# KyleVanMeter/MVOLPS

Hardware: AMD Instinct MI355X
Metric: simplex_pivots_per_s (higher is better)
Workload: dtype f64

## Files before the change

### include/mvx.h

```cpp
#ifndef MVX_H
#define MVX_H

#ifdef __cplusplus
extern "C" {
#endif

#define MVX_MIN 1
#define MVX_MAX 2
#define MVX_CV 1
#define MVX_IV 2
#define MVX_BV 3
#define MVX_FR 1
#define MVX_LO 2
#define MVX_UP 3
#define MVX_DB 4
#define MVX_FX 5
#define MVX_BS 1
#define MVX_NL 2
#define MVX_NU 3
#define MVX_NF 4
#define MVX_NS 5
#define MVX_UNDEF 1
#define MVX_FEAS 2
#define MVX_INFEAS 3
// ... 100 lines not shown
int mvx_price_cols(const mvx_prob *P, int k, const double *cols, const double *obj, double *dj, double *img);
int mvx_price_cols_tile(void);
void mvx_set_mat_col(mvx_prob *P, int j, int len, const int *ind, const double *val);
int mvx_get_mat_col(const mvx_prob *P, int j, int *ind, double *val);
int mvx_del_cols(mvx_prob *P, int ncs, const int *num);
int mvx_del_cols_span(void);
int mvx_conflict_graph(const mvx_prob *model, unsigned long long *adj, long long *edges);
int mvx_polish_many(const mvx_prob *root, int count, double *x, int max_moves, double *obj, int *moves, int *ok);

int mvx_get_tableau_ld(const mvx_prob *P);
int mvx_get_tableau(const mvx_prob *P, double *out);
int mvx_get_basis(const mvx_prob *P, int *head, int *nb, int *flag);

int mvx_device_count(void);
int mvx_set_device(int dev);
void mvx_profile_enable(int on);
void mvx_profile_reset(void);
double mvx_profile_update_ms(void);
long long mvx_profile_update_launches(void);
double mvx_last_solve_ms(const mvx_prob *P);
long long mvx_pack_size(const mvx_prob *P);
int mvx_pack(const mvx_prob *P, void *dev_buf);
long long mvx_pack_size_from(const mvx_prob *P, const mvx_prob *base);
int mvx_pack_from(const mvx_prob *P, const mvx_prob *base, void *dev_buf);
int mvx_unpack(mvx_prob *dst, const mvx_prob *base, const void *dev_buf);
void mvx_set_tuning(int tr, int hot, int nt);
void mvx_set_refresh(int check_every, double tol);
int mvx_get_refresh_cnt(const mvx_prob *P);
double mvx_row_residual(const mvx_prob *P);
void mvx_set_persist(int mode);
void mvx_set_chain(int len);
void mvx_set_cluster(int on);
void mvx_cluster_stats(long long *launches, long long *aborts);
void mvx_set_dual_chain(int len);
void mvx_persist_stats(long long *launches, long long *aborts);
void mvx_persist_cycles(unsigned long long *out5);
void mvx_set_batch_slots(int slots);
void mvx_sync(void);
int mvx_last_error(void);
int mvx_bind_thread(void);

#ifdef __cplusplus
}
#endif
#endif
```

### mvolps_amd/__init__.py

```python
import ctypes as C
import os

from . import capi

_HERE = os.path.dirname(os.path.abspath(__file__))
LIB_PATH = os.path.join(_HERE, "lib", "libmvolps_amd.so")

_EXTRA = {
    "del_rows": (C.c_int, [C.c_void_p, C.c_int, C.POINTER(C.c_int)]),
    "del_rows_many": (C.c_int, [C.c_void_p, C.c_int, C.POINTER(C.c_int), C.POINTER(C.c_int)]),
    "add_cut_rows_many": (C.c_int, [C.c_void_p, C.c_int, C.POINTER(C.c_int), C.POINTER(C.c_double), C.POINTER(C.c_double)]),
    "ranges": (C.c_int, [C.c_void_p, C.POINTER(C.c_double), C.POINTER(C.c_int)]),
    "ranges_chunk": (C.c_int, []),
    "add_dense_cols": (C.c_int, [C.c_void_p, C.c_int, C.POINTER(C.c_double), C.POINTER(C.c_double), C.POINTER(C.c_int),
                                 C.POINTER(C.c_double), C.POINTER(C.c_double), C.POINTER(C.c_int)]),
    "price_cols": (C.c_int, [C.c_void_p, C.c_int, C.POINTER(C.c_double), C.POINTER(C.c_double), C.POINTER(C.c_double),
                             C.POINTER(C.c_double)]),
    "price_cols_tile": (C.c_int, []),
    "del_cols": (C.c_int, [C.c_void_p, C.c_int, C.POINTER(C.c_int)]),
    "del_cols_span": (C.c_int, []),
    "set_mat_col": (None, [C.c_void_p, C.c_int, C.c_int, C.POINTER(C.c_int), C.POINTER(C.c_double)]),
    "get_mat_col": (C.c_int, [C.c_void_p, C.c_int, C.POINTER(C.c_int), C.POINTER(C.c_double)]),
    "device_count": (C.c_int, []),
    "set_device": (C.c_int, [C.c_int]),
    "profile_enable": (None, [C.c_int]),
    "profile_reset": (None, []),
    "profile_update_ms": (C.c_double, []),
    "profile_update_launches": (C.c_longlong, []),
    "last_solve_ms": (C.c_double, [C.c_void_p]),
    "sync": (None, []),
    "set_tuning": (None, [C.c_int, C.c_int, C.c_int]),
    "set_batch_slots": (None, [C.c_int]),
    "set_persist": (None, [C.c_int]),
    "set_chain": (None, [C.c_int]),
    "set_cluster": (None, [C.c_int]),
    "cluster_stats": (None, [C.POINTER(C.c_longlong), C.POINTER(C.c_longlong)]),
    "set_dual_chain": (None, [C.c_int]),
    "set_refresh": (None, [C.c_int, C.c_double]),
    "get_refresh_cnt": (C.c_int, [C.c_void_p]),
    "row_residual": (C.c_double, [C.c_void_p]),
    "persist_stats": (None, [C.POINTER(C.c_longlong), C.POINTER(C.c_longlong)]),
    "last_error": (C.c_int, []),
    "bind_thread": (C.c_int, []),
    "persist_cycles": (None, [C.POINTER(C.c_ulonglong)]),
    "simplex_batch": (C.c_int, [C.POINTER(C.c_void_p), C.c_int, C.c_void_p, C.POINTER(C.c_int)]),
    "pack_size": (C.c_longlong, [C.c_void_p]),
    "pack": (C.c_int, [C.c_void_p, C.c_void_p]),
    "pack_size_from": (C.c_longlong, [C.c_void_p, C.c_void_p]),
    "pack_from": (C.c_int, [C.c_void_p, C.c_void_p, C.c_void_p]),
    "unpack": (C.c_int, [C.c_void_p, C.c_void_p, C.c_void_p]),
}

_api = None


def load_library():
    if os.environ.get("MVX_NO_TORCH") != "1":
        try:
            import torch
        except Exception:
            pass
    if not os.path.exists(LIB_PATH):
        raise RuntimeError(
            "libmvolps_amd.so is missing (%s): build it with `python -m mvolps_amd.build`; "
            "there is no fallback path" % LIB_PATH
        )
    return C.CDLL(LIB_PATH)


# ... 19 lines not shown
```

### mvolps_amd/csrc/capi.cpp

```cpp
#include <algorithm>
#include <cfloat>
#include <cmath>
#include <cstdio>
#include <cstdlib>
#include <chrono>
#include <cstring>

#include "engine.hpp"
#include "../../include/mvx_dist.h"

using mvx::RowPtr;

static const double INF = HUGE_VAL;
static int g_term_out = 1;

static void fault(const char *msg) {
  std::fprintf(stderr, "mvx: %s\n", msg);
  std::abort();
}

static void norm_bounds(int type, double lb, double ub, double *olb, double *oub) {
  switch (type) {
    case MVX_FR: *olb = -INF; *oub = INF; break;
    case MVX_LO: *olb = lb; *oub = INF; break;
// ... 722 lines not shown
int mvx_conflict_graph(const mvx_prob *model, unsigned long long *adj, long long *edges) {
  return mvx::engine_conflict_graph(model, adj, edges);
}
int mvx_polish_many(const mvx_prob *root, int count, double *x, int max_moves, double *obj, int *moves, int *ok) {
  return mvx::engine_polish_many(root, count, x, max_moves, obj, moves, ok);
}

int mvx_device_count(void) { return mvx::device_count(); }
int mvx_set_device(int dev) { return mvx::set_device(dev); }
long long mvx_pack_size(const mvx_prob *P) { return mvx::engine_pack_size(P, P->m); }
int mvx_pack(const mvx_prob *P, void *dev_buf) { return mvx::engine_pack(P, P->m, dev_buf); }
long long mvx_pack_size_from(const mvx_prob *P, const mvx_prob *base) { return mvx::engine_pack_size(P, base ? base->m : P->m); }
int mvx_pack_from(const mvx_prob *P, const mvx_prob *base, void *dev_buf) { return mvx::engine_pack(P, base ? base->m : P->m, dev_buf); }
int mvx_unpack(mvx_prob *dst, const mvx_prob *base, const void *dev_buf) {
  if (dst == base) return -1;
  mvx::release_device(dst);
  dst->m = base->m; dst->n = base->n; dst->dir = base->dir;
  dst->A = base->A; dst->c = base->c; dst->kind = base->kind; dst->cname = base->cname;
  dst->rtype = base->rtype; dst->rlb = base->rlb; dst->rub = base->rub;
  dst->ctype = base->ctype; dst->clb = base->clb; dst->cub = base->cub;
  dst->valid = false; dst->sol_fresh = false; dst->fresh_rows = -1;
  return mvx::engine_unpack(dst, dev_buf);
}
void mvx_set_tuning(int tr, int hot, int nt) { mvx::tuning(tr, hot, nt); }
void mvx_set_stall_limit(int limit) { mvx::set_stall_limit(limit); }
int mvx_fcs_debug_stamps(unsigned long long *out) { return mvx::fcs_debug_stamps(out); }
void mvx_set_refresh(int check_every, double tol) { mvx::set_refresh(check_every, tol); }
int mvx_get_refresh_cnt(const mvx_prob *P) { return P->refresh_cnt; }
double mvx_row_residual(const mvx_prob *P) { return mvx::row_residual(P); }
void mvx_set_persist(int mode) { mvx::set_persist(mode); }
void mvx_set_chain(int len) { mvx::set_chain(len); }
void mvx_set_cluster(int on) { mvx::set_cluster(on); }
void mvx_cluster_stats(long long *launches, long long *aborts) { mvx::cluster_stats(launches, aborts); }
void mvx_set_dual_chain(int len) { mvx::set_dual_chain(len); }
void mvx_persist_stats(long long *launches, long long *aborts) { mvx::persist_stats(launches, aborts); }
void mvx_persist_cycles(unsigned long long *out5) { mvx::persist_cycles(out5); }
void mvx_set_batch_slots(int slots) { mvx::set_batch_slots(slots); }
void mvx_profile_enable(int on) { mvx::profile_enable(on); }
void mvx_profile_reset(void) { mvx::profile_reset(); }
double mvx_profile_update_ms(void) { return mvx::profile_update_ms(); }
long long mvx_profile_update_launches(void) { return mvx::profile_update_launches(); }
double mvx_last_solve_ms(const mvx_prob *P) { return P->last_ms; }
void mvx_sync(void) { mvx::sync_stream(); }
int mvx_last_error(void) { return mvx::take_last_error(); }
int mvx_bind_thread(void) { return mvx::bind_thread(); }

void *mvx_image_alloc(size_t bytes) { return mvx::engine_image_alloc(bytes); }
void mvx_image_free(void *buf) { mvx::engine_image_free(buf); }
static long long img_pack_size(const void *P, const void *base) { return mvx_pack_size_from((const mvx_prob *)P, (const mvx_prob *)base); }
static int img_pack(const void *P, const void *base, void *buf) { return mvx_pack_from((const mvx_prob *)P, (const mvx_prob *)base, buf); }
static int img_unpack(void *dst, const void *base, const void *buf) { return mvx_unpack((mvx_prob *)dst, (const mvx_prob *)base, buf); }
const mvx_image_api *mvx_hip_image_api(void) {
  static const mvx_image_api t = {img_pack_size, img_pack, img_unpack, mvx_image_alloc, mvx_image_free};
  return &t;
}

}
```

### mvolps_amd/csrc/engine.cpp

```cpp
#include <hip/hip_runtime.h>

#include <algorithm>
#include <cmath>
#include <cstdio>
#include <cstdlib>
#include <cstring>
#include <atomic>
#include <functional>
#include <limits>
#include <map>
#include <mutex>
#include <tuple>
#include <unordered_map>
#include <unordered_set>
#include <vector>

#include "engine.hpp"

struct DevMatrix {
  int m0 = 0, n = 0, lda = 0;
  double *plain = nullptr, *packed = nullptr;
  int *len = nullptr;
  std::vector<const void *> rows;
  ~DevMatrix() {
// ... 637 lines not shown
    *ub = P->rub[k];
  } else {
    *lb = P->clb[k - P->m];
    *ub = P->cub[k - P->m];
  }
}

static std::atomic<int> g_cluster{-1};
static std::atomic<bool> g_cluster_broken{false};
static std::atomic<long long> g_cluster_launches{0}, g_cluster_aborts{0};
static bool cluster_wanted() {
  int v = g_cluster.load();
  if (v < 0) {
    const char *e = std::getenv("MVX_CLUSTER");
    v = e ? (std::atoi(e) != 0) : 1;
    g_cluster.store(v);
  }
  return v != 0 && !g_cluster_broken.load();
}

static int g_chain = -1;
static int chain_length(const mvx_prob *P) {
  if (g_chain < 0) {
    const char *e = std::getenv("MVX_CHAIN");
    g_chain = e ? std::max(1, std::min(KCH, std::atoi(e))) : 0;
  }
  if (g_chain > 0) return g_chain;
  const size_t bytes = (size_t)(P->m + 1) * (size_t)P->ld * 8;
  if (cluster_wanted() && chain_cluster_kmax(P->m, P->n) > 0) return bytes < ((size_t)24 << 20) ? 16 : 32;
  if (bytes < ((size_t)24 << 20)) return 8;
  return 16;
}

static int g_dchain = -1;
static int dual_chain_length(bool wide, bool on_chip = false) {
  if (g_dchain < 0) {
    const char *e = std::getenv("MVX_DCHAIN");
    g_dchain = e ? std::max(1, std::min(DCH_MAX, std::atoi(e))) : 0;
  }
  if (g_dchain > 0) return g_dchain;
  if (on_chip) return 8;
  return wide ? 8 : 4;
}

static int pivot_budget(const mvx_prob *P, const mvx_smcp &parm) {
  return parm.it_lim >= 0 ? parm.it_lim : 200 * (P->m + P->n) + 100000;
}

static void ctl_for_handle(Ctl *h, const mvx_prob *P, double tol_bnd, double tol_dj, double tol_piv, int budget) {
  std::memset(h, 0, sizeof(Ctl));
  h->T = P->d_T;
  h->bvar = P->d_bvar; h->blb = P->d_blb; h->bub = P->d_bub;
  h->nvar = P->d_nvar; h->nflag = P->d_nflag; h->nlb = P->d_nlb; h->nub = P->d_nub;
  h->m = P->m; h->n = P->n; h->ld = P->ld; h->m_cap = P->m_cap;
  h->sgn = (P->dir == MVX_MAX) ? 1.0 : -1.0;
  h->tol_bnd = tol_bnd; h->tol_dj = tol_dj; h->tol_piv = tol_piv;
  h->phase = PH_START; h->done = D_RUN; h->budget = budget;
  h->stall = 0; h->stall_limit = g_stall_limit > 0 ? g_stall_limit : 64 + (P->m + P->n) / 8;
  h->fstate = F_OFF;
  h->nch = 1;
}

static void fill_ctl(SolveCtx &sc, mvx_prob *P, Ctl *h, const mvx_smcp *parm = nullptr) {
  if (parm) ctl_for_handle(h, P, parm->tol_bnd, parm->tol_dj, parm->tol_piv, pivot_budget(P, *parm));
  else ctl_for_handle(h, P, 1e-9, 1e-9, 1e-9, -1);
  h->colq = sc.d_colq; h->srow = sc.d_srow; h->cost1 = sc.d_cost1; h->wts = sc.d_wts;
// ... 132 lines not shown
        double acc = 0.0;
        if (any_x)
          for (int j = 1; j <= n; j++)
            if (xn[j] != 0.0) acc = std::fma(a[j], xn[j], acc);
        row[0] = acc;
      }
    }
    HIPCHECK(hipMemcpyAsync(P->d_T + r0 * ld, bounce, (r1 - r0) * ld * 8, hipMemcpyHostToDevice, sc.stream));
    HIPCHECK(hipStreamSynchronize(sc.stream));
  }
  HIPCHECK(hipHostFree(bounce));
  HIPCHECK(hipMemcpyAsync(P->d_bvar, P->bvar.data(), (size_t)(m + 1) * 4, hipMemcpyHostToDevice, sc.stream));
  HIPCHECK(hipMemcpyAsync(P->d_blb, blb.data(), (size_t)(m + 1) * 8, hipMemcpyHostToDevice, sc.stream));
  HIPCHECK(hipMemcpyAsync(P->d_bub, bub.data(), (size_t)(m + 1) * 8, hipMemcpyHostToDevice, sc.stream));
  std::vector<int> nv((size_t)ld, 0), nf((size_t)ld, MVX_NS);
  for (int j = 1; j <= n; j++) {
    nv[j] = P->nvar[j];
    nf[j] = P->nflag[j];
  }
  HIPCHECK(hipMemcpyAsync(P->d_nvar, nv.data(), (size_t)ld * 4, hipMemcpyHostToDevice, sc.stream));
  HIPCHECK(hipMemcpyAsync(P->d_nflag, nf.data(), (size_t)ld * 4, hipMemcpyHostToDevice, sc.stream));
  HIPCHECK(hipMemcpyAsync(P->d_nlb, nlb.data(), (size_t)ld * 8, hipMemcpyHostToDevice, sc.stream));
  HIPCHECK(hipMemcpyAsync(P->d_nub, nub.data(), (size_t)ld * 8, hipMemcpyHostToDevice, sc.stream));
  HIPCHECK(hipStreamSynchronize(sc.stream));
  rebuild_pos(P);
  P->pending.clear();
  P->valid = true;
  P->sol_fresh = false;
  P->fresh_rows = -1;
  P->status = MVX_UNDEF;
  return true;
}

static void flush_update_events(Context &c, size_t used) {
  for (size_t k = 0; k + 1 < used; k += 2) {
    float ms = 0.f;
    HIPCHECK(hipEventElapsedTime(&ms, c.ev_pool[k], c.ev_pool[k + 1]));
    c.prof_update_ms += ms;
    c.prof_update_n++;
  }
}

constexpr int PERSIST_HEAD_STRIDE_MAX = 4;
static std::atomic<int> g_persist_mode{-1};
static std::atomic<bool> g_persist_broken{false};
static std::atomic<long long> g_persist_launches{0}, g_persist_aborts{0};
struct PersistPlan {
  int cpw = 0, nw = 0;
  size_t lds = 0;
};
static bool persist_plan(Context &c, const mvx_prob *P, PersistPlan *pl) {
  if (g_persist_broken) return false;
  if (g_persist_mode < 0) {
    const char *e = std::getenv("MVX_PERSIST");
    g_persist_mode = (e && e[0] == '0') ? 0 : ((e && e[0] == '2') ? 2 : 1);
  }
  if (!g_persist_mode) return false;
  static int cus = 0;
  if (!cus) {
    hipDeviceProp_t prop;
    if (hipGetDeviceProperties(&prop, c.dev) != hipSuccess) return false;
    cus = prop.multiProcessorCount;
  }
  const int m = P->m, n = P->n;
  if ((long)(m + 1) * (n + 1) < 32768) return false;
  if (g_persist_mode < 2 && (long)(m + 1) * (n + 1) > 700000) return false;
  const int cpw = (n + cus - 1) / cus;
  if (cpw > persist_max_cpw()) return false;
// ... 14 lines not shown
    HIPCHECK(hipMalloc((void **)&sc.d_pcand, (size_t)2 * 256 * PERSIST_HEAD_STRIDE_MAX * 8));
    HIPCHECK(hipMalloc((void **)&sc.d_pctl, sizeof(Ctl)));
  }
  if (words > sc.p_msg_words) {
    HIPCHECK(hipStreamSynchronize(sc.stream));
    if (sc.d_pmsg) HIPCHECK(hipFree(sc.d_pmsg));
    HIPCHECK(hipMalloc((void **)&sc.d_pmsg, (size_t)2 * 256 * words * 8));
    sc.p_msg_words = words;
  }
  if (P->ld > sc.p_pw_ld) {
    HIPCHECK(hipStreamSynchronize(sc.stream));
    if (sc.d_ppw) HIPCHECK(hipFree(sc.d_ppw));
    HIPCHECK(hipMalloc((void **)&sc.d_ppw, (size_t)2 * P->ld * 8));
    sc.p_pw_ld = P->ld;
  }
  if (sc.p_backup_bytes != P->slab_bytes) {
    if (sc.p_backup) slab_recycle(c, sc.p_backup, sc.p_backup_bytes);
    sc.p_backup = slab_alloc(c, P->slab_bytes);
    sc.p_backup_bytes = sc.p_backup ? P->slab_bytes : 0;
    if (!sc.p_backup) {
      (void)g_last_error.exchange(0);
      return false;
    }
  }
  return true;
}

struct SolveJob {
  mvx_prob *P = nullptr;
  SolveCtx *sc = nullptr;
  mvx_smcp parm;
  enum { MAIN, PHASE1, FINAL } mode = MAIN;
  int batch = 8, pb = 4;
  int done = D_RUN;
  bool try_fused = false;
  bool try_dfused = false;
  bool persist_queued = false;
  int seen_steps = 0, seen_pivots = 0, seen_bulk = 0;
  int chain = 1, chain0 = 1;
  bool resident = false;
  bool cluster = false;
  ChainArgs cargs{};
  size_t ev_used = 0;
  bool profiled = false;
  int rc = 0;
  Ctl snap;
};

static void stage_copy_async(SolveCtx &sc, const mvx_prob *P) {
  HIPCHECK(hipEventRecord(sc.ev_b, sc.stream));
  if (!sc.stage_zc) HIPCHECK(hipMemcpyAsync(sc.h_stage, sc.d_stage, StageView::bytes(P->m_cap, P->ld), hipMemcpyDeviceToHost, sc.stream));
  if (sc.d_pabort) HIPCHECK(hipMemcpyAsync(sc.h_pabort, sc.d_pabort, 512, hipMemcpyDeviceToHost, sc.stream));
}

static bool dual_fused_worth_it(const mvx_prob *P) {
  static int mode = -1;
  if (mode < 0) {
    const char *e = std::getenv("MVX_DUAL_FUSED");
    mode = e ? std::atoi(e) : 1;
  }
  if (mode == 0) return false;
  if (mode >= 2) return true;
  const long entries = (long)(P->m + 1) * (P->n + 1);
  return entries >= 2000000 && entries < 12000000;
}

// ... 3 lines not shown
  ensure_scratch(sc, P->m_cap, P->ld);
  Ctl *h = sc.h_ctl;
  fill_ctl(sc, P, h, &J.parm);
  take_edits(P, h);
  upload_ctl(sc);
  HIPCHECK(hipEventRecord(sc.ev_a, sc.stream));
  {
    ChainArgs &a = J.cargs;
    a.c = sc.d_ctl;
    a.T = P->d_T;
    a.blb = P->d_blb; a.bub = P->d_bub; a.nlb = P->d_nlb; a.nub = P->d_nub; a.nflag = P->d_nflag;
    a.betab = sc.d_betab;
    for (int k = 0; k < 2; k++) {
      a.pw[k] = sc.d_pw[k];
      a.drowk[k] = sc.d_drowk[k]; a.pwk[k] = sc.d_pwk[k]; a.nlbk[k] = sc.d_nlbk[k]; a.nubk[k] = sc.d_nubk[k]; a.nflagk[k] = sc.d_nflagk[k];
      a.betak[k] = sc.d_betak[k]; a.blbk[k] = sc.d_blbk[k]; a.bubk[k] = sc.d_bubk[k];
    }
    a.pp = sc.d_ppart; a.rp = sc.d_rpart; a.ppstride = sc.pp_stride; a.rpstride = sc.rp_stride;
    a.srow0 = sc.d_srowk[0]; a.colq0 = sc.d_colqk[0];
    a.sstride = sc.sk_stride; a.cstride = sc.ck_stride;
    a.m = P->m; a.n = P->n; a.ld = P->ld; a.mcap1 = P->m_cap + 1;
    a.ncb = chain_ncb(P->n); a.nrb = chain_nrb(P->m);
    a.tol_dj = h->tol_dj; a.tol_piv = h->tol_piv; a.tol_bnd = h->tol_bnd; a.sgn = h->sgn;
    a.stall_limit = h->stall_limit;
    a.zeros = sc.d_zeros;
    a.xg = sc.d_xg; a.xg_bytes = (int)XG_BYTES; a.xabort = sc.d_xabort;
    a.nw = chain_cluster_nw(P->m, P->n); a.kmax = 0; a.tagbase = 0; a.boot = 0;
  }
  J.cluster = J.resident && cluster_wanted() && chain_cluster_kmax(P->m, P->n) > 0;
  J.try_fused = !P->hint_dual;
  J.chain = J.chain0 = h->chain_max;
  J.try_dfused = P->hint_dual && dual_fused_worth_it(P);
  J.profiled = c.prof && J.sc == &c.main;
  if (J.parm.it_lim > 8 && J.try_fused) J.batch = std::min(J.parm.it_lim, 256);
}

static void job_enqueue(Context &c, SolveJob &J) {
  mvx_prob *P = J.P;
  SolveCtx &sc = *J.sc;
  const int m = P->m, n = P->n;
  J.ev_used = 0;
  if (J.mode == SolveJob::FINAL) {
    launch_export(sc.d_ctl, sc.d_stage, m, n, 1, sc.stream);
    stage_copy_async(sc, P);
    return;
  }
  if (J.mode == SolveJob::PHASE1) {
    for (int k = 0; k < J.pb; k++) {
      launch_p1_head(sc.d_ctl, sc.stream);
      launch_p1_fix(sc.d_ctl, n, sc.stream);
      launch_p1_select(sc.d_ctl, sc.stream);
      launch_update(sc.d_ctl, m + 1, n, sc.stream);
    }
    launch_export(sc.d_ctl, sc.d_stage, m, n, 0, sc.stream);
    stage_copy_async(sc, P);
    return;
  }
  const int batch = J.batch;
  if (J.profiled && c.ev_pool.size() < (size_t)2 * batch + 4) {
    size_t old = c.ev_pool.size();
    c.ev_pool.resize((size_t)2 * batch + 4);
    for (size_t k = old; k < c.ev_pool.size(); k++) HIPCHECK(hipEventCreate(&c.ev_pool[k]));
  }
  const int remaining = (J.parm.it_lim >= 0) ? std::max(0, J.parm.it_lim - J.seen_pivots) : (1 << 30);
  auto ev = [&]() {
    if (J.profiled) HIPCHECK(hipEventRecord(c.ev_pool[J.ev_used++], sc.stream));
  };
  int depth;
  if (J.try_fused) depth = std::max(0, std::min(batch, remaining));
  else depth = std::max(1, std::min(batch, remaining));
  if (J.try_fused) {
    PersistPlan pl;
    if (depth > 0 && !J.profiled && J.resident && !(J.cluster && !g_cluster_broken.load()) && persist_plan(c, P, &pl) && ensure_persist(c, sc, P)) {
      launch_select(sc.d_ctl, sc.stream);
      launch_update(sc.d_ctl, m, n, sc.stream, 1, 1);
      HIPCHECK(hipMemcpyAsync(sc.p_backup, P->slab, P->slab_bytes, hipMemcpyDeviceToDevice, sc.stream));
      HIPCHECK(hipMemcpyAsync(sc.d_pctl, sc.d_ctl, sizeof(Ctl), hipMemcpyDeviceToDevice, sc.stream));
      HIPCHECK(hipMemcpyAsync(sc.d_ppw, sc.d_pw[0], (size_t)P->ld * 8, hipMemcpyDeviceToDevice, sc.stream));
      HIPCHECK(hipMemcpyAsync(sc.d_ppw + P->ld, sc.d_pw[1], (size_t)P->ld * 8, hipMemcpyDeviceToDevice, sc.stream));
      const int head_stride = 4;
      HIPCHECK(hipMemsetAsync(sc.d_pcand, 0, (size_t)2 * pl.nw * head_stride * 8, sc.stream));
      const int steps = 1 << 24;
      if (launch_persist(sc.d_ctl, sc.d_pcand, sc.d_pmsg, sc.d_pabort, (unsigned long long *)(sc.d_pabort + 16), P->m, pl.cpw, pl.nw, sc.p_msg_words, steps, head_stride, sc.stream) == 0) {
        J.persist_queued = true;
        g_persist_launches++;
        launch_select(sc.d_ctl, sc.stream);
        launch_update(sc.d_ctl, m, n, sc.stream, 1, 1);
      } else {
        g_persist_broken = true;
      }
    } else {
      const size_t e_generic = J.ev_used;
      if (J.profiled) J.ev_used += 2;
      if (depth > 0) {
        const bool cl = J.cluster && !g_cluster_broken.load();
        if (!cl) launch_pboot(J.cargs, sc.stream);
        bool first = true;
        const int kc = cl ? std::max(1, std::min(J.chain0, chain_cluster_kmax(m, n))) : std::max(1, J.chain);
        auto chain_launch = [&](int steps) {
          J.cargs.kmax = steps;
          J.cargs.boot = first ? 1 : 0;
          first = false;
          J.cargs.tagbase = sc.xtag;
          sc.xtag += 128;
          if (launch_chain(J.cargs, sc.stream) != 0) g_cluster_broken.store(true);
          g_cluster_launches++;
        };
        for (int left = depth; left > 0;) {
          const int steps = std::min(kc, left);
          if (cl) chain_launch(steps);
          else
            for (int t = 0; t < steps; t++) launch_pstep(J.cargs, t, sc.stream);
          ev();
          launch_fbc3(J.cargs, steps, sc.stream);
          ev();
          left -= steps;
        }
        if (J.parm.it_lim >= 0 && depth >= remaining && !cl) launch_pc(J.cargs, 0, sc.stream);
      }
      launch_select(sc.d_ctl, sc.stream);
      if (J.profiled) HIPCHECK(hipEventRecord(c.ev_pool[e_generic], sc.stream));
      launch_update(sc.d_ctl, m, n, sc.stream, 1, 1);
      if (J.profiled) HIPCHECK(hipEventRecord(c.ev_pool[e_generic + 1], sc.stream));
    }
  } else if (J.try_dfused) {
    launch_select(sc.d_ctl, sc.stream);
    launch_update(sc.d_ctl, m, n, sc.stream, 1, 1);
    if (depth > 1) {
      launch_dboot(sc.d_ctl, n, sc.stream);
      launch_db(sc.d_ctl, m, n, sc.stream);
      for (int k = 0; k < depth - 1; k++) {
        launch_da(sc.d_ctl, n, sc.stream);
        launch_db(sc.d_ctl, m, n, sc.stream);
      }
    }
  } else {
    for (int k = 0; k < depth; k++) {
      launch_dsel(sc.d_ctl, m, n, sc.stream);
      launch_select(sc.d_ctl, sc.stream);
      ev();
      launch_update(sc.d_ctl, m, n, sc.stream, 1, 1);
      ev();
    }
  }
  launch_export(sc.d_ctl, sc.d_stage, m, n, 0, sc.stream);
  stage_copy_async(sc, P);
}

static int book_result(mvx_prob *P, const Ctl &snap, int done, double last_ms) {
  P->it_cnt += snap.it_cnt;
  P->bland_cnt += snap.n_bland;
// ... 29 lines not shown
      mvx_prob *P = J.P;
      g_persist_broken = true;
      g_persist_aborts++;
      std::fprintf(stderr, "mvx: resident-tableau launch aborted (workgroups not co-resident in time); using the two-kernel path from now on\n");
      HIPCHECK(hipMemcpyAsync(P->slab, sc.p_backup, P->slab_bytes, hipMemcpyDeviceToDevice, sc.stream));
      HIPCHECK(hipMemcpyAsync(sc.d_ctl, sc.d_pctl, sizeof(Ctl), hipMemcpyDeviceToDevice, sc.stream));
      HIPCHECK(hipMemcpyAsync(sc.d_pw[0], sc.d_ppw, (size_t)P->ld * 8, hipMemcpyDeviceToDevice, sc.stream));
      HIPCHECK(hipMemcpyAsync(sc.d_pw[1], sc.d_ppw + P->ld, (size_t)P->ld * 8, hipMemcpyDeviceToDevice, sc.stream));
      HIPCHECK(hipMemsetAsync(sc.d_pabort, 0, sizeof(int), sc.stream));
      sc.h_pabort[0] = 0;
      J.try_fused = true;
      return false;
    }
  }
  std::memcpy(&snap, sc.h_stage, sizeof(Ctl));
  if (J.mode == SolveJob::FINAL) return job_finalize(J);
  if (J.mode == SolveJob::PHASE1) {
    if (snap.done == D_RUN) {
      J.pb = std::min(J.pb * 2, 64);
      return false;
    }
    if (snap.done == D_PFEAS) {
      snap.rounds++;
      if (snap.rounds >= 64) {
        J.done = D_FAIL;
        J.mode = SolveJob::FINAL;
        return false;
      }
      snap.done = D_RUN;
      snap.phase = PH_START;
      *sc.h_ctl = snap;
      upload_ctl(sc);
      J.mode = SolveJob::MAIN;
      J.batch = 8;
      J.try_fused = false;
      J.try_dfused = false;
      return false;
    }
    J.done = snap.done;
    return job_finalize(J);
  }
  if (J.profiled) {
    const int steps_now = snap.n_bulk;
    flush_update_events(c, std::min(J.ev_used, (size_t)2 * (size_t)(steps_now - J.seen_steps)));
    J.seen_steps = steps_now;
  }
  if (snap.cl_abort) {
    g_cluster_broken.store(true);
    g_cluster_aborts++;
    std::fprintf(stderr, "mvx: cluster selection launch aborted (peer workgroups not reachable in time); using two launches per chained step from now on\n");
    HIPCHECK(hipMemsetAsync(sc.d_xabort, 0, sizeof(int), sc.stream));
  }
  J.done = snap.done;
  {
    const int dp = snap.it_cnt - J.seen_pivots, db = snap.n_bulk - J.seen_bulk;
    if (J.chain0 > 1 && db >= 4) {
      if (2 * dp < J.chain * db) J.chain = std::max(1, J.chain / 2);
      else if (10 * dp >= 9 * J.chain * db) J.chain = std::min(J.chain0, J.chain * 2);
    }
    J.seen_bulk = snap.n_bulk;
  }
  J.seen_pivots = snap.it_cnt;
  J.try_fused = (snap.phase == PH_PRIMAL2) && snap.stall < snap.stall_limit;
  J.try_dfused = (snap.phase == PH_DUAL) && snap.stall < snap.stall_limit && dual_fused_worth_it(J.P);
  if (J.done == D_NEED_PHASE1) {
    snap.done = D_RUN;
    snap.phase = PH_PHASE1;
    snap.p1_init = 1;
    snap.p1_fix_q = 0;
    *sc.h_ctl = snap;
    upload_ctl(sc);
    J.mode = SolveJob::PHASE1;
    J.pb = 4;
    return false;
  }
  if (J.done != D_RUN) return job_finalize(J);
  J.batch = std::min(J.batch * 2, 256);
  return false;
}

static bool already_solved(const mvx_prob *P, const mvx_smcp &parm) {
  if (!P->valid || parm.it_lim == 0) return false;
  if (P->status != MVX_OPT) return false;
  return P->last_tol[0] == parm.tol_bnd && P->last_tol[1] == parm.tol_dj && P->last_tol[2] == parm.tol_piv;
}
static void remember_tolerances(mvx_prob *P, const mvx_smcp &parm) {
  P->last_tol[0] = parm.tol_bnd;
  P->last_tol[1] = parm.tol_dj;
  P->last_tol[2] = parm.tol_piv;
}

static bool admit(mvx_prob *P, const mvx_smcp &parm, int *rc) {
  if (P->m < 1 || P->n < 1) {
    P->status = MVX_UNDEF;
    *rc = MVX_EFAIL;
    return false;
  }
  if (already_solved(P, parm)) {
    P->last_ms = 0.0;
    *rc = 0;
    return false;
  }
  if (!P->valid && !build_slack_tableau(P)) {
    *rc = MVX_EFAIL;
    return false;
  }
  remember_tolerances(P, parm);
  P->fresh_rows = -1;
  return true;
}
// ... 2156 lines not shown
    HIPCHECK(hipMemcpyAsync(dst->d_T, d + h.host_bytes, tb, hipMemcpyDeviceToDevice, sc.stream));
    HIPCHECK(hipMemcpyAsync((unsigned char *)slab + L.o_bvar, d + h.host_bytes + align_up(tb, 256), L.total - L.o_bvar,
                            hipMemcpyDeviceToDevice, sc.stream));
    HIPCHECK(hipStreamSynchronize(sc.stream));
    rebuild_pos(dst);
    dst->valid = true;
  }
  return 0;
}

void tuning(int tr, int hot, int nt) {
  sync_stream();
  set_tuning(tr, hot, nt);
  if (g_ctx) {
    g_ctx->main.sc_m_cap = 0;
    g_ctx->main.sc_ld = 0;
  }
}

void set_dual_chain(int len) { g_dchain = (len <= 0) ? 0 : std::min(DCH_MAX, len); }
void set_chain(int len) { g_chain = (len <= 0) ? 0 : std::min(KCH, len); }
void set_cluster(int on) {
  g_cluster.store(on != 0);
  g_cluster_broken.store(false);
}
void cluster_stats(long long *launches, long long *aborts) {
  *launches = g_cluster_launches.load();
  *aborts = g_cluster_aborts.load();
}
void set_persist(int mode) {
  g_persist_mode = mode < 0 ? -1 : (mode > 2 ? 2 : mode);
  g_persist_broken = false;
}
void persist_stats(long long *launches, long long *aborts) {
  *launches = g_persist_launches;
  *aborts = g_persist_aborts;
}
void persist_cycles(unsigned long long *out5) {
  for (int k = 0; k < 48; k++) out5[k] = 0;
  if (!g_ctx || !g_ctx->main.h_pabort) return;
  const unsigned long long *d = (const unsigned long long *)(g_ctx->main.h_pabort + 16);
  for (int k = 0; k < 48; k++) out5[k] = d[k];
}
int fcs_debug_stamps(unsigned long long *out) {
  Context &c = ctx();
  if (!c.main.h_ctl || !c.main.h_ctl->dbg) return 0;
  HIPCHECK(hipDeviceSynchronize());
  HIPCHECK(hipMemcpy(out, c.main.h_ctl->dbg, (size_t)KCH * 16 * 8, hipMemcpyDeviceToHost));
  return KCH;
}
void set_stall_limit(int limit) { g_stall_limit = limit > 0 ? limit : 0; }
void set_batch_slots(int k) { g_batch_slots = k < 2 ? 2 : (k > 256 ? 256 : k); }
void profile_enable(int on) { ctx().prof = on != 0; }
void profile_reset() {
  Context &c = ctx();
  MAIN_LOCK(c);
  c.prof_update_ms = 0.0;
  c.prof_update_n = 0;
}
double profile_update_ms() { return g_ctx ? g_ctx->prof_update_ms : 0.0; }
long long profile_update_launches() { return g_ctx ? g_ctx->prof_update_n : 0; }

}
```

### mvolps_amd/csrc/engine.hpp

```cpp
#pragma once
#include "mvx_internal.hpp"

namespace mvx {

int device_count();
int set_device(int dev);
void sync_stream();
int take_last_error();
int bind_thread();

int engine_simplex(mvx_prob *P, const mvx_smcp *parm);
int engine_simplex_batch(mvx_prob **probs, int count, const mvx_smcp *parm, int *rcs);

void engine_apply_bounds(mvx_prob *P, int k, int type, double old_lb, double old_ub, double lb, double ub);
void engine_add_rows(mvx_prob *P, int first, int nrs);
void engine_del_rows(mvx_prob *P, const std::vector<int> &rows, int m_old);
void engine_del_rows_many(mvx_prob *const *Ps, int count, const std::vector<int> *rows, const int *m_old);
void engine_row_from_model(mvx_prob *P, int i);
void engine_recompute_cost_row(mvx_prob *P);
void engine_invalidate(mvx_prob *P);

void engine_copy(mvx_prob *dst, const mvx_prob *src);
void release_device(mvx_prob *P);

// ... 11 lines not shown
int engine_round_many(const mvx_prob *root, const mvx_prob *const *Ps, int count, int mode, double *obj, int *found, double *x);
int engine_dive_pick_many(const mvx_prob *root, const mvx_prob *const *Ps, int count, const int *rules, int *nfrac, int *col, int *dir,
                          double *val);
int engine_set_obj_many(mvx_prob *const *Ps, int count, const double *c);
int engine_pump_obj_many(const mvx_prob *root, const mvx_prob *const *Ps, int count, const double *xprev, const int *has_prev,
                         const double *ab, int *info, double *xt, double *c);
int engine_cut_scores(const mvx_prob *P, int k, const double *vals, const double *x, double *dot, double *gram);
int engine_add_cut_rows(mvx_prob *P, int k, const double *vals, const double *rhs);
int engine_add_cut_rows_many(mvx_prob *const *Ps, int count, const int *off, const double *vals, const double *rhs);
int engine_add_cols_live(mvx_prob *P, int k, const double *cols, const double *obj, const int *flag, const double *lb, const double *ub);
int engine_price_cols(const mvx_prob *P, int k, const double *cols, const double *obj, double *dj, double *img);
int engine_del_cols(mvx_prob *P, const std::vector<int> &cols, int n_old, const double *lb, const double *ub);
int engine_conflict_graph(const mvx_prob *R, unsigned long long *adj, long long *edges);
int engine_polish_many(const mvx_prob *root, int count, double *x, int max_moves, double *obj, int *moves, int *ok);
int engine_rc_tighten_many(const mvx_prob *const *Ps, int count, const double *cutoff, double tol, int *cnt, int *cols, double *lb,
                           double *ub);
int engine_tighten_many(mvx_prob *const *Ps, int count, const int *off, const int *cols, const double *lb, const double *ub);
int engine_propagate_many(const mvx_prob *root, const mvx_prob *const *Ps, int count, int max_rounds, int *infeasible, int *rounds, int *cnt,
                          int *cols, double *lb, double *ub);
int engine_set_bounds_many(mvx_prob *const *Ps, int count, const int *off, const int *cols, const double *lb, const double *ub);

long long engine_pack_size(const mvx_prob *P, int m_base);
int engine_pack(const mvx_prob *P, int m_base, void *dev_buf);
int engine_unpack(mvx_prob *dst, const void *dev_buf);
void *engine_image_alloc(size_t bytes);
void engine_image_free(void *p);
void tuning(int tr, int hot, int nt);
void set_stall_limit(int limit);
int fcs_debug_stamps(unsigned long long *out);
void set_persist(int mode);
void set_chain(int len);
void set_cluster(int on);
void cluster_stats(long long *launches, long long *aborts);
void set_dual_chain(int len);
void set_refresh(int check_every, double tol);
double row_residual(const mvx_prob *P);
void persist_stats(long long *launches, long long *aborts);
void persist_cycles(unsigned long long *out5);
void set_batch_slots(int k);
void profile_enable(int on);
void profile_reset();
double profile_update_ms();
long long profile_update_launches();

}
```

### mvolps_amd/csrc/kernels.hip

```cpp
#include <hip/hip_runtime.h>

#include <atomic>
#include <cmath>
#include <cstdlib>

#include "kernel_common.hpp"

namespace mvx {

template <int MODE>
__device__ __forceinline__ bool cand_better(const Cand &a, const Cand &b) {
  if (a.idx == 0) return false;
  if (b.idx == 0) return true;
  if (MODE == 0) {
    if (a.k1 > b.k1) return true;
    if (a.k1 < b.k1) return false;
    return a.idx < b.idx;
  } else {
    if (a.k1 < b.k1) return true;
    if (a.k1 > b.k1) return false;
    if (a.k2 > b.k2) return true;
    if (a.k2 < b.k2) return false;
    return a.idx < b.idx;
  }
// ... 796 lines not shown
      c->ch_piv[kk] = apq;
      c->ch_xq[kk] = xq;
      c->ch_s0[kk] = s0;
    }
    nch = kk + 1;
    DS_STAMP(4);
    if (stats && TIDX == 0) atomicAdd(&g_dsel_cycles[6], 1ull);
  }
#undef DC_HC
#undef DC_HS
  if (stats && TIDX == 0) atomicAdd(&g_round_hist[nch ? nch : DCH_MAX + 1], 1ull);
  if (nch == 0) return;
  if (ract) k.dw[i] = dw;
  if (t == 0) {
    c->stall = stall;
    c->nch = nch;
    c->dsel = 1;
    c->step = ST_PIVOT;
    c->p = p0;
    c->q = q0;
    c->p_up = p_up0;
    c->piv = piv0;
    c->bound = bound0;
    c->xq = xq0;
    c->leave_flag = lf0;
  }
  DS_STAMP(5);
  if (stats && TIDX == 0) atomicAdd(&g_dsel_cycles[7], 1ull);
#undef DS_STAMP
}

__device__ void select_step(Ctl *c, Cand *lds) {
  const KC k = load_kc(c);
  if (c->done != D_RUN) return;
  if (c->pc_itlim) {
    __syncthreads();
    if (TIDX == 0) {
      c->pc_itlim = 0;
      c->fstate = F_STOP;
    }
    dev_finish(c, D_ITLIM, PH_PRIMAL2, c->rounds);
    return;
  }
  if (TIDX == 0) c->nch = 1;
  const int ne = c->n_edits;
  if (ne) {
    if (TIDX < ne) {
      const int r = c->edit_row[TIDX];
      k.blb[r] = c->edit_lb[TIDX];
      k.bub[r] = c->edit_ub[TIDX];
    }
    __syncthreads();
    if (TIDX == 0) c->n_edits = 0;
  }
  int phase = c->phase, rounds = c->rounds;
  int nch = 1;
  int p = 0, p_up = 0, q = 0, sdir = 0, kind = 0;
  bool fresh_dual = false;
  bool fresh_primal = false;
  for (;;) {
    if (phase == PH_START) {
      Cand r = dev_infeas_row(k, lds, nullptr);
      if (r.idx == 0) {
        phase = PH_PRIMAL2;
        fresh_primal = true;
      } else {
        Cand pr = dev_price(k, k.T, k.sgn, lds);
        if (pr.idx != 0) {
          dev_finish(c, D_NEED_PHASE1, PH_PHASE1, rounds);
          return;
        }
        phase = PH_DUAL;
        p = r.idx;
        p_up = r.aux;
        kind = 2;
// ... 1224 lines not shown
  if (fnew != MVX_NS) {
    Cand x{0.0, 0.0, 0, 0};
    if (price_col(fnew, A.sgn * dnew, A.tol_dj, j, wnew, x)) best = x;
  }
  publish_pricing(A, best, b, dnew, wnew, lbj, ubj, fnew, s_slots, s_pay);
  PR_STAMP(4);
  if (act) {
    A.srow0[(size_t)g * A.sstride + j] = sj;
    A.drowk[xw][j] = dnew;
    A.pwk[xw][j] = (j >= 1) ? wnew : 1.0;
    A.nflagk[xw][j] = (j >= 1) ? fnew : MVX_NS;
    A.nlbk[xw][j] = lbj;
    A.nubk[xw][j] = ubj;
  }
  if (lead) {
    c->ch_kind[g] = kind;
    c->ch_p[g] = flip ? 0 : p;
    c->ch_q[g] = q;
    c->ch_lf[g] = lf;
    c->ch_piv[g] = flip ? 1.0 : piv;
    c->ch_xq[g] = xq;
    c->ch_s0[g] = s0;
    c->ch_delta[g] = delta;
    c->ch_elb[g] = lbq;
    c->ch_eub[g] = ubq;
    c->ch_llb[g] = plb;
    c->ch_lub[g] = pub;
    c->ch_bound[g] = bound;
    c->ch_pup[g] = p_up;
    c->ch_stall[g] = stall_new;
    c->ch_cnt[g] = used + (flip ? 0 : 1);
    c->ch_ok[g] = epoch;
    c->pc_n = g + 1;
  }
  PR_STAMP(5);
#undef PR_STAMP
}

constexpr int XNW = 64;
constexpr int XNF = 8;
enum : int { XAUX_SC0 = 1, XAUX_SC1 = 16 };
typedef unsigned xu4 __attribute__((ext_vector_type(4)));

struct XCtx {
  __amdgpu_buffer_rsrc_t rs;
  int w, nw;
  unsigned tag;
  int xno;
  int *xabort;
  bool dead;
  bool flag;
};

__device__ __forceinline__ double ld_sc1(const double *p) {
  return __longlong_as_double((long long)__hip_atomic_load(reinterpret_cast<const unsigned long long *>(p), __ATOMIC_RELAXED, __HIP_MEMORY_SCOPE_AGENT));
}

template <int MODE, int NP>
__device__ __forceinline__ Cand xchg(XCtx &X, Cand mine, const double (&pin)[NP], double (&pout)[NP], Cand (*s_slots)[4], double (*s_pay)[4][5]) {
  const int lane = TIDX & 63, wave = TIDX >> 6, b = X.xno & 1;
  int ol;
  Cand wb = wave_argbest<MODE>(mine, &ol);
  wb.aux = (wb.aux & 0xffff) | (__ballot(X.flag) ? 0x10000 : 0);
  if (lane == 0) s_slots[b][wave] = wb;
#pragma unroll
  for (int k = 0; k < NP; k++) {
// ... 81 lines not shown
  int stall = c->stall;
  const bool boot = (A.boot != 0);
  const bool fresh = boot && (phase0 == PH_START);
  const int fstate = boot ? F_RUN : fstate0;
  const bool boot_off = boot && (stall >= A.stall_limit || !(phase0 == PH_PRIMAL2 || (fresh && n_edits == 0)));
  double d[CPT], wgt[CPT], lbj[CPT], ubj[CPT], sqn[CPT];
  int f[CPT], jj[CPT];
#pragma unroll
  for (int u = 0; u < CPT; u++) {
    const int j = 1 + gt + u * TT;
    const bool act = (j <= n);
    const int jc = act ? j : n;
    jj[u] = j;
    d[u] = T[jc];
    wgt[u] = fresh ? 1.0 : A.pw[boot ? cur0 : 0][jc];
    f[u] = act ? A.nflag[jc] : MVX_NS;
    lbj[u] = A.nlb[jc];
    ubj[u] = A.nub[jc];
    sqn[u] = 0.0;
  }
  double z = T[0];
  double be[RPT], lb[RPT], ub[RPT];
  int ii[RPT];
#pragma unroll
  for (int u = 0; u < RPT; u++) {
    const int i = 1 + gt + u * TT;
    const int ic = (i <= m) ? i : m;
    ii[u] = i;
    be[u] = boot ? T[(size_t)ic * ld] : A.betab[ic];
    lb[u] = A.blb[ic];
    ub[u] = A.bub[ic];
  }
  if (done != D_RUN || fstate != F_RUN || aborted) return;
  if (boot_off) {
    if (lead) c->fstate = F_OFF;
    return;
  }
  XCtx X;
  X.rs = __builtin_amdgcn_make_buffer_rsrc(A.xg, 0, A.xg_bytes, 0x00027000);
  X.w = w;
  X.nw = nw;
  X.tag = A.tagbase + 1;
  X.xno = 0;
  X.xabort = A.xabort;
  X.dead = false;
  X.flag = false;
  if (fresh) {
    const double tolb = A.tol_bnd;
#pragma unroll
    for (int u = 0; u < RPT; u++) {
      if (ii[u] <= m) {
        if (lb[u] > -INFINITY && be[u] < lb[u] - tolb * (1.0 + fabs(lb[u]))) X.flag = true;
        if (ub[u] < INFINITY && be[u] > ub[u] + tolb * (1.0 + fabs(ub[u]))) X.flag = true;
      }
    }
  }
#define HS(S, U) hist[((size_t)(S) * (CPT + RPT) + (U)) * 256 + t]
#define HC(S, U) hist[((size_t)(S) * (CPT + RPT) + CPT + (U)) * 256 + t]
  int g = 0, used = 0;
  Cand pc;
  double pp[5], po[5];
#define PRICE()                                                                                          \
  do {                                                                                                   \
    pc = Cand{0.0, 0.0, 0, 0};                                                                           \
    pp[0] = d[0]; pp[1] = wgt[0]; pp[2] = lbj[0]; pp[3] = ubj[0]; pp[4] = sqn[0];                        \
    _Pragma("unroll") for (int u = 0; u < CPT; u++) {                                                    \
// ... 274 lines not shown
      c->pc_n = 0;
      c->cl_abort = 1;
    }
    return;
  }
  if (g == 0 && fresh) {
#pragma unroll
    for (int u = 0; u < CPT; u++) {
      if (jj[u] <= n) {
        A.pw[0][jj[u]] = 1.0;
        A.pw[1][jj[u]] = 1.0;
      }
    }
  }
  if (g > 0) {
    const int xf = g & 1;
#pragma unroll
    for (int u = 0; u < CPT; u++) {
      if (jj[u] <= n) {
        A.drowk[xf][jj[u]] = d[u];
        A.pwk[xf][jj[u]] = wgt[u];
      }
    }
    if (lead) {
      A.drowk[xf][0] = z;
      A.pwk[xf][0] = 1.0;
    }
  }
  if (lead) {
    c->pc_n = g;
    if (g > 0) {
      c->phase = PH_PRIMAL2;
      c->pc_itlim = end_itlim ? 1 : 0;
    }
  }
}

__device__ void chain_commit(const ChainArgs &A, Ctl *c, int nch) {
  __shared__ int s_cp[KCH], s_cq[KCH], s_ck[KCH], s_rf[KCH], s_cf[KCH], s_R[KCH], s_C[KCH];
  const int t = TIDX;
  const bool on = (t < nch);
  int kind = 0, p = 0, q = 0;
  if (on) {
    kind = c->ch_kind[t];
    p = c->ch_p[t];
    q = c->ch_q[t];
    s_ck[t] = kind;
    s_cp[t] = p;
    s_cq[t] = q;
    s_R[t] = (kind == ST_PIVOT) ? c->bvar[p] : 0;
    s_C[t] = (kind == ST_PIVOT) ? c->nvar[q] : 0;
  }
  __syncthreads();
  bool lastrow = true, lastcol = true, lastflag = true;
  if (on) {
    int rf = t, cf = t;
    for (int u = t - 1; u >= 0; u--) {
      if (s_ck[u] != ST_PIVOT) continue;
      if (s_cp[u] == p) rf = u;
      if (s_cq[u] == q) cf = u;
    }
    s_rf[t] = rf;
    s_cf[t] = cf;
    for (int u = t + 1; u < nch; u++) {
      if (s_cq[u] == q) lastflag = false;
      if (s_ck[u] != ST_PIVOT) continue;
// ... 1011 lines not shown
```

### mvolps_amd/csrc/mvx_internal.hpp

```cpp
#pragma once

#include <cstddef>
#include <cstdint>
#include <memory>
#include <string>
#include <vector>

#include <hip/hip_runtime_api.h>

#include "../../include/mvx.h"

struct DevMatrix;
namespace mvx {

constexpr int ROWCOMB_CHUNK = 64;
constexpr int LD_ALIGN = 32;
constexpr int ROW_SLACK = 64;
constexpr double DEGEN_TOL = 1e-9;
constexpr double PERT_EPS = 1e-6;
constexpr size_t NT_THRESHOLD_BYTES = (size_t)320 << 20;
constexpr size_t WT_MIN_BYTES = (size_t)96 << 20, WT_MAX_BYTES = (size_t)272 << 20;
constexpr int KCH = 32;
constexpr int DCH_MAX = 8;
constexpr int DA_THREADS = 1024;
// ... 39 lines not shown
  double *olb, *oub;
  int perturbed, pert_used, n_pert;
  int *p1_list;
  int p1_init, p1_nchg, p1_fix_q, p1_fix_g;
  double *pw[2];
  double *dw;
  int stall_new;
  double ent_lb, ent_ub;
  int n_edits, edit_row[MAX_EDITS];
  double edit_lb[MAX_EDITS], edit_ub[MAX_EDITS];
  int job;
  double *dwx[2];
  int p_nextx[2], p_up_nextx[2];
  int npbd;
  int chain_max, nch;
  int dchain_max;
  int n_bulk;
  int ch_alive, ch_nrpc;
  int ch_p[KCH], ch_q[KCH], ch_pup[KCH], ch_lf[KCH], ch_stall[KCH], ch_sdir[KCH], ch_fq[KCH];
  double ch_piv[KCH], ch_bound[KCH], ch_xq[KCH], ch_s0[KCH], ch_dq[KCH], ch_wq[KCH];
  Cand *rpc;
  double ch_elb[KCH], ch_eub[KCH];
  double ch_llb[KCH], ch_lub[KCH];
  double *srowk[KCH], *colqk[KCH];
  int pc_n;
  int pc_epoch;
  unsigned pc_arrive;
  int ch_kind[KCH], ch_cnt[KCH], ch_ok[KCH];
  int ch_okc[KCH];
  int hd_q[KCH], hd_sdir[KCH], hd_fq[KCH];
  double hd_dq[KCH], hd_wq[KCH], hd_lbq[KCH], hd_ubq[KCH];
  double ch_delta[KCH];
  int pc_itlim;
  int dsel;
  int cl_abort;
  unsigned long long *dbg;
};

struct StageView {
  double *beta, *dj;
  int *bvar, *nvar, *nflag;
  __host__ __device__ StageView(unsigned char *base, int m_cap, int ld) {
    beta = reinterpret_cast<double *>(base + sizeof(Ctl));
    dj = beta + (m_cap + 1);
    bvar = reinterpret_cast<int *>(dj + ld);
    nvar = bvar + (m_cap + 1);
    nflag = nvar + ld;
  }
  static size_t bytes(int m_cap, int ld) {
    return (sizeof(Ctl) + (size_t)(m_cap + 1) * (8 + 4) + (size_t)ld * (8 + 4 + 4) + 255) / 256 * 256;
  }
};

struct ChainArgs {
  Ctl *c;
  double *T;
  double *blb, *bub, *nlb, *nub;
  int *nflag;
  double *pw[2];
  double *betab;
  double *drowk[2], *pwk[2], *nlbk[2], *nubk[2];
  int *nflagk[2];
  double *betak[2], *blbk[2], *bubk[2];
  double *pp;
  double *rp;
  size_t ppstride, rpstride;
// ... 502 lines not shown
```

Before: 63210.

## Grow fused primal batch size with a separate cap and settle device-side chain continuation

Splits the host batch size into a generic batch and a fused-primal batch, the latter growing up to a configurable cap (default 1024) instead of the fixed 256. Adds a device-side pc_more flag so that when a chained primal run ends exactly at its step limit, the select kernel settles and returns instead of running a full selection, and the pc kernel is now always launched after non-cluster chains. The aim is fewer host round-trips and kernel-launch syncs per pivot. The cost is longer queued batches that may overshoot and extra device control state. Stats counters and an API knob are also added.

Measured after the change: 63130. No clear change (-0.1%).

```diff
diff --git a/include/mvx.h b/include/mvx.h
--- a/include/mvx.h
+++ b/include/mvx.h
@@ -156,6 +156,8 @@
 void mvx_set_chain(int len);
 void mvx_set_cluster(int on);
 void mvx_cluster_stats(long long *launches, long long *aborts);
+void mvx_set_primal_batch(int cap);
+void mvx_primal_batch_stats(long long *batches, long long *closing_pivots, long long *closing_settles);
 void mvx_set_dual_chain(int len);
 void mvx_persist_stats(long long *launches, long long *aborts);
 void mvx_persist_cycles(unsigned long long *out5);
diff --git a/mvolps_amd/__init__.py b/mvolps_amd/__init__.py
--- a/mvolps_amd/__init__.py
+++ b/mvolps_amd/__init__.py
@@ -35,6 +35,8 @@
     "set_chain": (None, [C.c_int]),
     "set_cluster": (None, [C.c_int]),
     "cluster_stats": (None, [C.POINTER(C.c_longlong), C.POINTER(C.c_longlong)]),
+    "set_primal_batch": (None, [C.c_int]),
+    "primal_batch_stats": (None, [C.POINTER(C.c_longlong), C.POINTER(C.c_longlong), C.POINTER(C.c_longlong)]),
     "set_dual_chain": (None, [C.c_int]),
     "set_refresh": (None, [C.c_int, C.c_double]),
     "get_refresh_cnt": (C.c_int, [C.c_void_p]),
diff --git a/mvolps_amd/csrc/capi.cpp b/mvolps_amd/csrc/capi.cpp
--- a/mvolps_amd/csrc/capi.cpp
+++ b/mvolps_amd/csrc/capi.cpp
@@ -778,6 +778,10 @@
 void mvx_set_chain(int len) { mvx::set_chain(len); }
 void mvx_set_cluster(int on) { mvx::set_cluster(on); }
 void mvx_cluster_stats(long long *launches, long long *aborts) { mvx::cluster_stats(launches, aborts); }
+void mvx_set_primal_batch(int cap) { mvx::set_primal_batch(cap); }
+void mvx_primal_batch_stats(long long *batches, long long *closing_pivots, long long *closing_settles) {
+  mvx::primal_batch_stats(batches, closing_pivots, closing_settles);
+}
 void mvx_set_dual_chain(int len) { mvx::set_dual_chain(len); }
 void mvx_persist_stats(long long *launches, long long *aborts) { mvx::persist_stats(launches, aborts); }
 void mvx_persist_cycles(unsigned long long *out5) { mvx::persist_cycles(out5); }
diff --git a/mvolps_amd/csrc/engine.cpp b/mvolps_amd/csrc/engine.cpp
--- a/mvolps_amd/csrc/engine.cpp
+++ b/mvolps_amd/csrc/engine.cpp
@@ -693,6 +693,20 @@
   return 16;
 }
 
+constexpr int PRIMAL_BATCH_DEFAULT = 1024;
+constexpr int PRIMAL_BATCH_MAX = 1 << 16;
+static std::atomic<int> g_primal_batch{0};
+static int primal_batch_cap() {
+  int v = g_primal_batch.load();
+  if (const char *e = std::getenv("MVX_PRIMAL_BATCH")) {
+    const int ev = std::atoi(e);
+    if (ev > 0) v = ev;
+  }
+  if (v <= 0) v = PRIMAL_BATCH_DEFAULT;
+  return std::min(v, PRIMAL_BATCH_MAX);
+}
+static std::atomic<long long> g_pb_batches{0}, g_pb_closing_pivots{0}, g_pb_closing_settles{0};
+
 static int g_dchain = -1;
 static int dual_chain_length(bool wide, bool on_chip = false) {
   if (g_dchain < 0) {
@@ -891,8 +905,8 @@
   return true;
 }
 
-static void flush_update_events(Context &c, size_t used) {
-  for (size_t k = 0; k + 1 < used; k += 2) {
+static void flush_update_events(Context &c, size_t first, size_t used) {
+  for (size_t k = first; k + 1 < used; k += 2) {
     float ms = 0.f;
     HIPCHECK(hipEventElapsedTime(&ms, c.ev_pool[k], c.ev_pool[k + 1]));
     c.prof_update_ms += ms;
@@ -973,6 +987,9 @@
   mvx_smcp parm;
   enum { MAIN, PHASE1, FINAL } mode = MAIN;
   int batch = 8, pb = 4;
+  int gbatch = 8, fbatch = 8, fcap = 256;
+  bool chained_queued = false;
+  int seen_settles = 0;
   int done = D_RUN;
   bool try_fused = false;
   bool try_dfused = false;
@@ -1042,7 +1059,11 @@
   J.chain = J.chain0 = h->chain_max;
   J.try_dfused = P->hint_dual && dual_fused_worth_it(P);
   J.profiled = c.prof && J.sc == &c.main;
-  if (J.parm.it_lim > 8 && J.try_fused) J.batch = std::min(J.parm.it_lim, 256);
+  J.fcap = primal_batch_cap();
+  J.gbatch = 8;
+  if (J.parm.it_lim > 8 && J.try_fused) J.gbatch = std::min(J.parm.it_lim, 256);
+  J.fbatch = (J.parm.it_lim >= 0) ? std::max(1, std::min(J.parm.it_lim, J.fcap)) : std::min(256, J.fcap);
+  J.batch = J.try_fused ? J.fbatch : J.gbatch;
 }
 
 static void job_enqueue(Context &c, SolveJob &J) {
@@ -1067,6 +1088,7 @@
     return;
   }
   const int batch = J.batch;
+  J.chained_queued = false;
   if (J.profiled && c.ev_pool.size() < (size_t)2 * batch + 4) {
     size_t old = c.ev_pool.size();
     c.ev_pool.resize((size_t)2 * batch + 4);
@@ -1103,6 +1125,7 @@
       const size_t e_generic = J.ev_used;
       if (J.profiled) J.ev_used += 2;
       if (depth > 0) {
+        J.chained_queued = true;
         const bool cl = J.cluster && !g_cluster_broken.load();
         if (!cl) launch_pboot(J.cargs, sc.stream);
         bool first = true;
@@ -1119,14 +1142,16 @@
         for (int left = depth; left > 0;) {
           const int steps = std::min(kc, left);
           if (cl) chain_launch(steps);
-          else
+          else {
+            J.cargs.kmax = steps;
             for (int t = 0; t < steps; t++) launch_pstep(J.cargs, t, sc.stream);
+          }
           ev();
           launch_fbc3(J.cargs, steps, sc.stream);
           ev();
           left -= steps;
         }
-        if (J.parm.it_lim >= 0 && depth >= remaining && !cl) launch_pc(J.cargs, 0, sc.stream);
+        if (!cl) launch_pc(J.cargs, 0, sc.stream);
       }
       launch_select(sc.d_ctl, sc.stream);
       if (J.profiled) HIPCHECK(hipEventRecord(c.ev_pool[e_generic], sc.stream));
@@ -1222,7 +1247,7 @@
       *sc.h_ctl = snap;
       upload_ctl(sc);
       J.mode = SolveJob::MAIN;
-      J.batch = 8;
+      J.batch = J.gbatch = 8;
       J.try_fused = false;
       J.try_dfused = false;
       return false;
@@ -1230,9 +1255,17 @@
     J.done = snap.done;
     return job_finalize(J);
   }
+  const bool settled = snap.n_settle != J.seen_settles;
+  J.seen_settles = snap.n_settle;
+  if (J.chained_queued) {
+    g_pb_batches++;
+    if (settled) g_pb_closing_settles++;
+    else if (snap.step == ST_PIVOT) g_pb_closing_pivots++;
+  }
   if (J.profiled) {
     const int steps_now = snap.n_bulk;
-    flush_update_events(c, std::min(J.ev_used, (size_t)2 * (size_t)(steps_now - J.seen_steps)));
+    const size_t first = settled ? 2 : 0;
+    flush_update_events(c, first, std::min(J.ev_used, first + (size_t)2 * (size_t)(steps_now - J.seen_steps)));
     J.seen_steps = steps_now;
   }
   if (snap.cl_abort) {
@@ -1265,7 +1298,9 @@
     return false;
   }
   if (J.done != D_RUN) return job_finalize(J);
-  J.batch = std::min(J.batch * 2, 256);
+  J.gbatch = std::min(J.gbatch * 2, 256);
+  if (J.chained_queued) J.fbatch = std::min(J.fbatch * 2, J.fcap);
+  J.batch = J.try_fused ? J.fbatch : J.gbatch;
   return false;
 }
 
@@ -3488,6 +3523,18 @@
   g_persist_mode = mode < 0 ? -1 : (mode > 2 ? 2 : mode);
   g_persist_broken = false;
 }
+void set_primal_batch(int cap) { g_primal_batch.store(cap > 0 ? cap : 0); }
+void primal_batch_stats(long long *batches, long long *closing_pivots, long long *closing_settles) {
+  if (!batches && !closing_pivots && !closing_settles) {
+    g_pb_batches.store(0);
+    g_pb_closing_pivots.store(0);
+    g_pb_closing_settles.store(0);
+    return;
+  }
+  if (batches) *batches = g_pb_batches.load();
+  if (closing_pivots) *closing_pivots = g_pb_closing_pivots.load();
+  if (closing_settles) *closing_settles = g_pb_closing_settles.load();
+}
 void persist_stats(long long *launches, long long *aborts) {
   *launches = g_persist_launches;
   *aborts = g_persist_aborts;
diff --git a/mvolps_amd/csrc/engine.hpp b/mvolps_amd/csrc/engine.hpp
--- a/mvolps_amd/csrc/engine.hpp
+++ b/mvolps_amd/csrc/engine.hpp
@@ -67,6 +67,8 @@
 void set_chain(int len);
 void set_cluster(int on);
 void cluster_stats(long long *launches, long long *aborts);
+void set_primal_batch(int cap);
+void primal_batch_stats(long long *batches, long long *closing_pivots, long long *closing_settles);
 void set_dual_chain(int len);
 void set_refresh(int check_every, double tol);
 double row_residual(const mvx_prob *P);
diff --git a/mvolps_amd/csrc/kernels.hip b/mvolps_amd/csrc/kernels.hip
--- a/mvolps_amd/csrc/kernels.hip
+++ b/mvolps_amd/csrc/kernels.hip
@@ -852,6 +852,7 @@
 
 __device__ void select_step(Ctl *c, Cand *lds) {
   const KC k = load_kc(c);
+  const int pc_more = c->pc_more;
   if (c->done != D_RUN) return;
   if (c->pc_itlim) {
     __syncthreads();
@@ -861,6 +862,18 @@
     }
     dev_finish(c, D_ITLIM, PH_PRIMAL2, c->rounds);
     return;
+  }
+  if (pc_more) {
+    const bool live = (c->fstate == F_RUN && c->phase == PH_PRIMAL2 && c->n_edits == 0);
+    __syncthreads();
+    if (TIDX == 0) c->pc_more = 0;
+    if (live) {
+      if (TIDX == 0) {
+        c->step = ST_NONE;
+        c->n_settle++;
+      }
+      return;
+    }
   }
   if (TIDX == 0) c->nch = 1;
   const int ne = c->n_edits;
@@ -2151,6 +2164,8 @@
     c->ch_cnt[g] = used + (flip ? 0 : 1);
     c->ch_ok[g] = epoch;
     c->pc_n = g + 1;
+    const int budget = c->budget;
+    c->pc_more = (g + 1 == A.kmax && stall_new < A.stall_limit && (budget < 0 || budget - (used + (flip ? 0 : 1)) > 0)) ? 1 : 0;
   }
   PR_STAMP(5);
 #undef PR_STAMP
@@ -2298,6 +2313,7 @@
     ub[u] = A.bub[ic];
   }
   if (done != D_RUN || fstate != F_RUN || aborted) return;
+  if (lead) c->pc_more = 0;
   if (boot_off) {
     if (lead) c->fstate = F_OFF;
     return;
@@ -2638,6 +2654,7 @@
     if (g > 0) {
       c->phase = PH_PRIMAL2;
       c->pc_itlim = end_itlim ? 1 : 0;
+      c->pc_more = (g >= kmax && qc.idx != 0 && (budget < 0 || budget - used > 0) && stall < A.stall_limit) ? 1 : 0;
     }
   }
 }
diff --git a/mvolps_amd/csrc/mvx_internal.hpp b/mvolps_amd/csrc/mvx_internal.hpp
--- a/mvolps_amd/csrc/mvx_internal.hpp
+++ b/mvolps_amd/csrc/mvx_internal.hpp
@@ -95,6 +95,8 @@
   double hd_dq[KCH], hd_wq[KCH], hd_lbq[KCH], hd_ubq[KCH];
   double ch_delta[KCH];
   int pc_itlim;
+  int pc_more;
+  int n_settle;
   int dsel;
   int cl_abort;
   unsigned long long *dbg;
```
